# Tony-Tseng/deep-rawburst-sr

Hardware: AMD Instinct MI355X
Metric: bursts/sec 14x48x48 RAW->4x (SyntheticBurstVal shape), DBSR forward (higher is better)
Workload: dtype fp16; 1 GPU; configs[1]: SyntheticBurstVal 14-frame 48x48 -> 384x384 (sr x8 of RAW, x4 of full-res), batch 8 per GPU, full PWC-Net + warp + fusion + decoder; global_batch=8, frames=14, height=48, width=48, out_size=384, parallelism=dp1 (independent bursts per rank), hip_graph=True, fusion_weights_written=True

## Files before the change

### deep-rawburst-sr_amd/csrc/conv2d.hip

```cpp
#include "conv_core.hpp"

#include <algorithm>
#include <type_traits>
#include <cstdlib>
#include <cstring>
#include <vector>

using namespace dbsr;

namespace {

int g_tiled_enabled = 1;

const dbsr_conv_desc* sel_view(const dbsr_conv_desc* d, dbsr_conv_desc& v) {
    if (d->plan_h <= 0 || d->plan_h == d->out_h) return d;
    v = *d;
    v.in_h = d->in_h + (d->plan_h - d->out_h) * d->stride;
    v.out_h = d->plan_h;
    return &v;
}

__host__ __device__ __forceinline__ int pipe_lane_ch(int cb, int h, int g, int cout) {
    const int c = cb + 32 * h + 8 * g;
    return c < cout ? c : cb;
// ... 1513 lines not shown
            asm volatile("ds_read_b128 %0, %1 offset:%2" : "=v"(v) : "v"(a), "i"(16 * (c * S::CH_U4 + 4 * imm)));
            bq[n % AHEAD].v = v;
        };
        auto epilogue = [&](auto y_) {
            constexpr int y = decltype(y_)::value;
            if (has_res) asm volatile("" : "+v"(resv[y]));
            if constexpr (has_gate) asm volatile("" : "+v"(gatev[y]));
            float v[8];
#pragma unroll
            for (int r = 0; r < 4; ++r) {
                v[r] = act1(acc[0][y][r] + bias0[r]);
                v[4 + r] = act1(acc[1][y][r] + bias1[r]);
            }
            if (has_res) {
#pragma unroll
                for (int e = 0; e < 4; ++e) {
                    v[2 * e] = act2(v[2 * e] + H16<T>::lo(resv[y][e]));
                    v[2 * e + 1] = act2(v[2 * e + 1] + H16<T>::hi(resv[y][e]));
                }
            }
            if constexpr (has_gate) {
#pragma unroll
                for (int e = 0; e < 4; ++e) {
                    v[2 * e] = H16<T>::lo(gatev[y][e]) > 0.f ? v[2 * e] : 0.f;
                    v[2 * e + 1] = H16<T>::hi(gatev[y][e]) > 0.f ? v[2 * e + 1] : 0.f;
                }
            }
            u32x4_t o;
#pragma unroll
            for (int e = 0; e < 4; ++e) o[e] = H16<T>::pack(v[2 * e], v[2 * e + 1]);
            __builtin_amdgcn_raw_buffer_store_b128(o, y_rsrc, cout_ok ? ys + y * ys_row : BUF_OOB, 0, 0);
        };

        StaticFor<0, AHEAD>::run([&](auto n_) { rd(n_); });
        StaticFor<0, S::READS>::run([&](auto n_) {
            constexpr int n = decltype(n_)::value, c = S::read_chunk(n);
            constexpr int newer = AHEAD - 1 < S::READS - 1 - n ? AHEAD - 1 : S::READS - 1 - n;
            bf16x8_t v = bq[n % AHEAD].v;
            asm volatile("s_waitcnt lgkmcnt(%1)" : "+v"(v) : "i"(newer));
            Frag<T> bf;
            bf.v = v;
            StaticFor<0, 3>::run([&](auto ky_) {
                constexpr int ky = decltype(ky_)::value;
                if constexpr (S::feeds(n, ky)) {
                    constexpr int y = S::read_row(n) - ky, tap = 3 * ky + S::read_kx(n);
                    const f32x4_t z = {0.f, 0.f, 0.f, 0.f};
                    acc[0][y] = mma(wr[c][tap][0], bf, S::kstep(n, ky) == 0 ? z : acc[0][y]);
                    acc[1][y] = mma(wr[c][tap][1], bf, S::kstep(n, ky) == 0 ? z : acc[1][y]);
                }
            });
            if constexpr (n + AHEAD < S::READS) rd(std::integral_constant<int, n + AHEAD>{});
            StaticFor<0, S::PER>::run([&](auto it_) {
                constexpr int it = decltype(it_)::value;
                if constexpr (n == S::dma_at(it)) {
                    if (more) dma(it, nxt, buf ^ 1);
                }
            });
            StaticFor<0, RPW>::run([&](auto y_) {
                constexpr int y = decltype(y_)::value;
                if constexpr (n == S::res_at(y)) {
                    if (has_res)
                        resv[y] = __builtin_amdgcn_raw_buffer_load_b128(
                            buf_rsrc((const T*)k.r + cur.r_off, rframe_bytes), r_tile + y * r_row, 0, 0);
                    if constexpr (has_gate)
                        gatev[y] = *(const u32x4_t*)((const T*)k.gt + cur.g_off + gl + y * g_row);
                }
                if constexpr (n == S::row_done(y)) epilogue(y_);
            });
        });
        PIPE_STAMP(7 + ti * 5);
        cur = nxt;
#pragma unroll
        for (int rho = 0; rho < 8; ++rho)
            ba[rho] += buf ? (unsigned)(-S::STAGE_U4 * 16) : (unsigned)(S::STAGE_U4 * 16);
    }
    vm_drain();
    PIPE_STAMP(1);
}

template <typename T, int WM, int TW, int TH, int NCH, int EPI>
__global__ __launch_bounds__(512, 1) void conv3x3_ws_kernel(ConvK k, int tiles_x, int tiles_y, int nct, int nsp,
                                                            int px) {
    constexpr bool rows = WM == wsr::WM && !(TH == 16 && NCH == 2 && (EPI == 0 || EPI == 5));
    if constexpr (rows) {
        static_assert(TW == wsr::TW, "the 64-cout tiles are 16 pixels wide");
        ws_rows_body<T, TH, NCH, EPI>(k, tiles_x, tiles_y, nct, nsp, px);
    } else {
        ws_tile_body<T, WM, TW, TH, NCH, EPI>(k, tiles_x, tiles_y, nct, nsp, px);
    }
}

int g_ws_enabled = 1;
inline bool ws_narrow(const dbsr_conv_desc* d) { return d->cout <= 32; }
inline bool ws_short(const dbsr_conv_desc* d) {
    if (d->gate.ptr && d->cout > 32 && d->cin > 32) return true;
    return !ws_narrow(d) && d->cin > 32 && d->out_w % 16 == 0 && d->out_h % 16 == 0 &&
           (long long)d->n_frames * (d->out_w / 16) * (d->out_h / 16) * ((d->cout + 63) / 64) < 128;
}
int pick_ws(const dbsr_conv_desc* d, const dbsr_conv_desc* g) {
    if (!g_ws_enabled || !conv3x3_16(d) || !slices_aligned8(d) || d->cin <= 16 || d->cin > 64 || d->cout % 8 ||
        d->cout > 512)
        return 0;
    const bool narrow = ws_narrow(d);
    const int tw = narrow ? 64 : 16, th = (narrow || ws_short(d)) ? 8 : 16, wm = narrow ? 32 : 64;
    if (narrow && (d->cout < 16 || d->cin > 32)) return 0;
    if (d->out_w % tw || d->out_h % th) return 0;
    if ((long long)d->in_h * d->in_w * d->x.ld * 2 >= (1LL << 31)) return 0;
    if (d->res.ptr && (long long)d->out_h * d->out_w * d->res.ld * 2 >= (1LL << 31)) return 0;
    if (!narrow && 16LL * d->out_w * d->y.ld * 2 >= (1LL << 31)) return 0;
    const int nct = (d->cout + wm - 1) / wm;
    const long long nsp = (long long)d->n_frames * (d->out_w / tw) * (d->out_h / th);
    const int cus = d->max_blocks > 0 ? std::min(d->max_blocks, num_cus()) : num_cus();
    if (cus / 8 / nct < 1 || nsp * nct < 64) return 0;
    if (g->out_h % th) return -1;
    const long long nsp_g = (long long)g->n_frames * (g->out_w / tw) * (g->out_h / th);
    const long long want = (nsp_g + 7) / 8;
    const long long spx = std::max<long long>(1, std::min<long long>(cus / 8 / nct, want));
    return (int)(spx * nct);
}

template <typename T, int WM, int TW, int TH, int NCH>
int launch_ws(const ConvK& k, const dbsr_conv_desc* d, int px, hipStream_t s) {
    const int tiles_x = k.out_w / TW, tiles_y = k.out_h / TH;
    const int nct = (k.cout + WM - 1) / WM;
    const int nsp = d->n_frames * tiles_x * tiles_y;
#define DBSR_WS_LAUNCH(E)                                                                                       \
    hipLaunchKernelGGL((conv3x3_ws_kernel<T, WM, TW, TH, NCH, E>), dim3(8 * px), dim3(512), 0, s, k, tiles_x,    \
                       tiles_y, nct, nsp, px)
    switch (epi_code(k)) {
        case 1: DBSR_WS_LAUNCH(1); break;
        case 2: DBSR_WS_LAUNCH(2); break;
        case 3: DBSR_WS_LAUNCH(3); break;
        case 5: DBSR_WS_LAUNCH(5); break;
        default: DBSR_WS_LAUNCH(0); break;
    }
#undef DBSR_WS_LAUNCH
    DBSR_LAUNCH_CHECK();
    return 0;
}

int g_ks128_enabled = 1;
bool use_ks128(const dbsr_conv_desc* d) {
    if (!g_ks128_enabled || !conv3x3_16(d) || !slices_aligned8(d) || cin_pad(d->cin) != 128 || d->cout != 128)
        return false;
    if (d->out_w % ks128::TW || d->out_h % ks128::TH || (d->plan_h > 0 && d->plan_h != d->out_h)) return false;
    if ((long long)d->in_h * d->in_w * d->x.ld * 2 >= (1LL << 31)) return false;
    return (long long)d->n_frames * (d->out_w / ks128::TW) * (d->out_h / ks128::TH) >= 128;
}
int launch_ks128(const ConvK& k, const dbsr_conv_desc* d, hipStream_t s) {
    return ks128_launch(k, d->n_frames, d->x.dtype == DBSR_F16, epi_code(k), k.max_blocks, num_cus(), s);
}

namespace rbk {
constexpr int TW = 32, TH = 16;
constexpr int MW = TW + 2, MH = TH + 2, MPX = MW * MH;
constexpr int IW = TW + 4, IH = TH + 4, IPX = IW * IH;
constexpr int IN_PIECES = (IPX + 15) / 16;
constexpr int IN_U4 = IN_PIECES * 64;
constexpr int G1 = (MPX + 15) / 16;
constexpr int MID_U4 = G1 * 16 * 4;
constexpr int G2 = TW * TH / 16;
constexpr int NW = 8;
constexpr int PER = (IN_PIECES + NW - 1) / NW;
constexpr int Q1 = (G1 + NW - 1) / NW;
constexpr int Q2 = G2 / NW;
constexpr int NG = 2;
constexpr int LDS_BYTES = (2 * IN_U4 + MID_U4) * 16 + 64 * 4;
static_assert(LDS_BYTES <= 160 * 1024, "resblock LDS");
}

template <typename T, bool HEAD>
__global__ __launch_bounds__(512, 1) void resblock32_kernel(ConvK k1, ConvK k2, int tiles_x, int tiles_y,
                                                            int ntiles) {
    using namespace rbk;
    DBSR_OWN_SIMDS();
    __shared__ __attribute__((aligned(16))) u32x4_t lds[2 * IN_U4 + MID_U4 + 16 + 34];
    u32x4_t* lmid = lds + 2 * IN_U4;
    float* lbias = (float*)(lds + 2 * IN_U4 + MID_U4);
    float* lhead = lbias + 64;
    const int lane = threadIdx.x & 63, wave = __builtin_amdgcn_readfirstlane(threadIdx.x >> 6);
    const int H = k1.in_h, W = k1.in_w;

    Frag<T> w1[9][2], w2[9][2];
#pragma unroll
    for (int tap = 0; tap < 9; ++tap)
#pragma unroll
        for (int h = 0; h < 2; ++h) {
            w1[tap][h].load((const T*)((const char*)k1.w_pipe + (h * 9 + tap) * 1024 + lane * 16));
            w2[tap][h].load((const T*)((const char*)k2.w_pipe + (h * 9 + tap) * 1024 + lane * 16));
        }
    if (threadIdx.x < 64) {
        const ConvK& kb = threadIdx.x < 32 ? k1 : k2;
        lbias[threadIdx.x] = kb.bias ? kb.bias[threadIdx.x & 31] : 0.f;
    }
    if constexpr (HEAD) {
        if (threadIdx.x < 128) lhead[threadIdx.x] = (int)threadIdx.x < k2.head_cout * 32 ? k2.head_w[threadIdx.x] : 0.f;
        if (threadIdx.x < 4)
            lhead[128 + threadIdx.x] = (k2.head_b && (int)threadIdx.x < k2.head_cout) ? k2.head_b[threadIdx.x] : 0.f;
    }

    struct Tile { const T* xf; long long y_off; int y0, x0; };
    auto decode = [&](int i) {
        const int t = rb_tile(i, blockIdx.x, gridDim.x, ntiles);
        Tile tl;
        const int tx = t % tiles_x, r = t / tiles_x, ty = r % tiles_y, f = r / tiles_y;
        tl.y0 = ty * TH; tl.x0 = tx * TW;
        tl.xf = (const T*)k1.x + map_frame(k1.xm, f) * k1.x_is;
        tl.y_off = HEAD ? map_frame(k2.ym, f) * k2.y_is + (long long)tl.y0 * W + tl.x0
                        : map_frame(k2.ym, f) * k2.y_is + k2.y_c0 + ((long long)tl.y0 * W + tl.x0) * k2.y_ld;
        return tl;
    };
    const int my_tiles = ntiles / (int)gridDim.x + ((int)blockIdx.x < ntiles % (int)gridDim.x ? 1 : 0);
    const int pix_b = k1.x_ld * (int)sizeof(T);
    const unsigned frame_bytes = (unsigned)((long long)H * W * pix_b);
    const unsigned lds0 = (unsigned)(unsigned long long)(__attribute__((address_space(3))) u32x4_t*)lds;
    auto dma = [&](const Tile& tl, int buf) {
        int ln = lane;
        asm volatile("" : "+v"(ln));
#pragma unroll
        for (int it = 0; it < PER; ++it) {
            const int piece = min(wave + NW * it, IN_PIECES - 1);
            const int p = piece * 16 + (ln >> 2), ph = ln & 3;
            const int gg = 2 * ((ph & 1) ^ ((p >> 2) & 1)) + (ph >> 1);
            const int r = p / IW, c = p - r * IW;
            const int hy = tl.y0 - 2 + r, hx = tl.x0 - 2 + c;
            const bool ok = p < IPX && (unsigned)hy < (unsigned)H && (unsigned)hx < (unsigned)W;
            lds_dma16(tl.xf, frame_bytes, ok ? (hy * W + hx) * pix_b + gg * 16 : BUF_OOB, 0,
                      lds0 + (buf * IN_U4 + piece * 64) * 16);
        }
    };

    auto taps = [&](const u32x4_t* img, int iw, int g, const auto& P0, const Frag<T> (&w)[9][2], auto& acc) {
        constexpr int NB = std::extent<std::remove_reference_t<decltype(P0)>>::value;
        int bs[NB][8];
#pragma unroll
        for (int j = 0; j < NB; ++j)
#pragma unroll
            for (int rho = 0; rho < 8; ++rho) bs[j][rho] = 4 * P0[j] + halo_phys(P0[j] + rho, g);
        Frag<T> bq[NB][3];
        auto rd = [&](int j, int tap) {
            const int imm = (tap / 3) * iw + tap % 3;
            Frag<T> b;
            b.v = __builtin_bit_cast(bf16x8_t, img[bs[j][imm & 7] + 4 * imm]);
            return b;
        };
#pragma unroll
        for (int j = 0; j < NB; ++j) {
            bq[j][0] = rd(j, 0);
            bq[j][1] = rd(j, 1);
        }
        StaticFor<0, 9>::run([&](auto t_) {
            constexpr int tap = decltype(t_)::value;
            const f32x4_t z = {0.f, 0.f, 0.f, 0.f};
#pragma unroll
            for (int j = 0; j < NB; ++j) {
                acc[j][0] = mma(w[tap][0], bq[j][tap % 3], tap == 0 ? z : acc[j][0]);
                acc[j][1] = mma(w[tap][1], bq[j][tap % 3], tap == 0 ? z : acc[j][1]);
                if constexpr (tap + 2 < 9) bq[j][(tap + 2) % 3] = rd(j, tap + 2);
            }
        });
        __builtin_amdgcn_iglp_opt(0);
    };

    auto store_out = [&](const Tile& tl, int i, int g, int col, const u32x4_t& o) {
        const int q = wave + NW * i;
        const long long px = (long long)(q >> 1) * W + 16 * (q & 1) + col;
        if constexpr (HEAD) {
            if (g < k2.head_cout) ((float*)k2.y)[tl.y_off + px + (long long)g * H * W] = __uint_as_float(o[0]);
        } else {
            *(u32x4_t*)((T*)k2.y + tl.y_off + px * k2.y_ld + 8 * g) = o;
        }
    };
    Tile cur = decode(0), prev = cur;
    if (my_tiles > 0) dma(cur, 0);
    u32x4_t outv[Q2];
    for (int ti = 0; ti < my_tiles; ++ti) {
        dma_barrier();
        int ln = lane;
        asm volatile("" : "+v"(ln));
        const int g = ln >> 4, col = ln & 15;
        if (ti > 0) {
#pragma unroll
            for (int i = 0; i < Q2; ++i) store_out(prev, i, g, col, outv[i]);
        }
        const u32x4_t* lin = lds + (ti & 1) * IN_U4;
        const bool more = ti + 1 < my_tiles;
        const Tile nxt = more ? decode(ti + 1) : cur;
        if (more) dma(nxt, (ti + 1) & 1);
        {
            const float4 b0 = *(const float4*)(lbias + 8 * g), b1 = *(const float4*)(lbias + 8 * g + 4);
            const float bv[8] = {b0.x, b0.y, b0.z, b0.w, b1.x, b1.y, b1.z, b1.w};
            auto conv1 = [&](auto nb_, auto q0_) {
                constexpr int NB = decltype(nb_)::value, Q0 = decltype(q0_)::value;
                int pa[NB], P0[NB];
#pragma unroll
                for (int j = 0; j < NB; ++j) {
                    pa[j] = min(16 * (wave + NW * (Q0 + j)) + col, MPX - 1);
                    const int r = pa[j] / MW, c = pa[j] - r * MW;
                    P0[j] = r * IW + c;
                }
                f32x4_t acc[NB][2];
                taps(lin, IW, g, P0, w1, acc);
#pragma unroll
                for (int j = 0; j < NB; ++j) {
                    const int p = 16 * (wave + NW * (Q0 + j)) + col;
                    const int r = pa[j] / MW, c = pa[j] - r * MW;
                    const int fy = cur.y0 - 1 + r, fx = cur.x0 - 1 + c;
                    const bool inside = (unsigned)fy < (unsigned)H && (unsigned)fx < (unsigned)W;
                    u32x4_t o;
#pragma unroll
                    for (int e = 0; e < 2; ++e) {
                        o[e] = relu16x2(H16<T>::pack(acc[j][0][2 * e] + bv[2 * e], acc[j][0][2 * e + 1] + bv[2 * e + 1]));
                        o[2 + e] = relu16x2(H16<T>::pack(acc[j][1][2 * e] + bv[4 + 2 * e],
                                                         acc[j][1][2 * e + 1] + bv[4 + 2 * e + 1]));
                    }
                    if (!inside) o = u32x4_t{0u, 0u, 0u, 0u};
                    if (p < MPX) lmid[4 * p + halo_phys(p, g)] = o;
                }
            };
            StaticFor<0, Q1 / NG>::run([&](auto bt_) {
                conv1(std::integral_constant<int, NG>{}, std::integral_constant<int, NG * decltype(bt_)::value>{});
            });
            if constexpr (Q1 % NG != 0) {
                if (wave + NW * (Q1 - Q1 % NG) < G1)
                    conv1(std::integral_constant<int, Q1 % NG>{}, std::integral_constant<int, Q1 - Q1 % NG>{});
            }
        }
        dma_barrier();
        {
            const float4 b0 = *(const float4*)(lbias + 32 + 8 * g), b1 = *(const float4*)(lbias + 32 + 8 * g + 4);
            const float bv[8] = {b0.x, b0.y, b0.z, b0.w, b1.x, b1.y, b1.z, b1.w};
            StaticFor<0, Q2 / NG>::run([&](auto bt_) {
                constexpr int bt = decltype(bt_)::value;
                int row[NG], cc[NG], P0[NG];
#pragma unroll
                for (int j = 0; j < NG; ++j) {
                    const int q = wave + NW * (NG * bt + j);
                    row[j] = q >> 1;
                    cc[j] = 16 * (q & 1) + col;
                    P0[j] = row[j] * MW + cc[j];
                }
                f32x4_t acc[NG][2];
                taps(lmid, MW, g, P0, w2, acc);
#pragma unroll
                for (int j = 0; j < NG; ++j) {
                    const int PR = (row[j] + 2) * IW + cc[j] + 2;
                    const u32x4_t rq = lin[4 * PR + halo_phys(PR, g)];
                    float v[8];
#pragma unroll
                    for (int r = 0; r < 4; ++r) {
                        v[r] = acc[j][0][r] + bv[r];
                        v[4 + r] = acc[j][1][r] + bv[4 + r];
                    }
                    u32x4_t o;
                    if constexpr (HEAD) {
#pragma unroll
                        for (int e = 0; e < 4; ++e) {
                            v[2 * e] = fmaxf(v[2 * e] + H16<T>::lo(rq[e]), 0.f);
                            v[2 * e + 1] = fmaxf(v[2 * e + 1] + H16<T>::hi(rq[e]), 0.f);
                        }
                        float hs[4];
#pragma unroll
                        for (int c = 0; c < 4; ++c) {
                            const float4 w0 = *(const float4*)(lhead + c * 32 + 8 * g);
                            const float4 w1 = *(const float4*)(lhead + c * 32 + 8 * g + 4);
                            float a = v[0] * w0.x;
                            a = fmaf(v[1], w0.y, a); a = fmaf(v[2], w0.z, a); a = fmaf(v[3], w0.w, a);
                            a = fmaf(v[4], w1.x, a); a = fmaf(v[5], w1.y, a); a = fmaf(v[6], w1.z, a);
                            a = fmaf(v[7], w1.w, a);
                            a += __shfl_xor(a, 16, 64);
                            a += __shfl_xor(a, 32, 64);
                            hs[c] = a;
                        }
                        const float hv = g == 0 ? hs[0] : g == 1 ? hs[1] : g == 2 ? hs[2] : hs[3];
                        o = u32x4_t{__float_as_uint(fmaxf(hv + lhead[128 + g], 0.f)), 0u, 0u, 0u};
                    } else {
#pragma unroll
                        for (int e = 0; e < 4; ++e)
                            o[e] = relu16x2(H16<T>::pack(v[2 * e] + H16<T>::lo(rq[e]), v[2 * e + 1] + H16<T>::hi(rq[e])));
                    }
                    outv[NG * bt + j] = o;
                }
            });
        }
        prev = cur;
        cur = nxt;
    }
    if (my_tiles > 0) {
#pragma unroll
        for (int i = 0; i < Q2; ++i) store_out(prev, i, lane >> 4, lane & 15, outv[i]);
    }
    vm_drain();
}

void tensor_span(const dbsr_tensor& t, int n, long long per_img, int es, unsigned long long& lo,
                 unsigned long long& hi) {
    long long mn = 0, mx = 0;
    for (int f = 0; f < n; ++f) {
        const long long img = (long long)(f / t.map.fpg) * t.map.group_stride + t.map.group_offset +
                              (long long)(f % t.map.fpg) * t.map.inner_stride;
        if (f == 0 || img < mn) mn = img;
        if (f == 0 || img > mx) mx = img;
    }
    const unsigned long long base = (unsigned long long)(uintptr_t)t.ptr;
    lo = base + (unsigned long long)((mn * t.img_stride + t.c0) * es);
    hi = base + (unsigned long long)((mx * t.img_stride + per_img) * es);
}
bool resblock_out_disjoint(const dbsr_conv_desc* c1, const dbsr_conv_desc* c2, const dbsr_tensor* head_out,
                           int head_cout) {
    const long long hw = (long long)c1->in_h * c1->in_w;
    const int C = c1->cin;
    unsigned long long xl, xh, yl, yh;
    tensor_span(c1->x, c1->n_frames, (hw - 1) * c1->x.ld + c1->x.c0 + C, 2, xl, xh);
    if (head_out) tensor_span(*head_out, c1->n_frames, (long long)head_cout * hw, 4, yl, yh);
    else tensor_span(c2->y, c1->n_frames, (hw - 1) * c2->y.ld + c2->y.c0 + C, 2, yl, yh);
    return yh <= xl || xh <= yl;
}

int resblock_channels(const dbsr_conv_desc* c1, const dbsr_conv_desc* c2) {
    if (!c1 || !c2) return 0;
    const int C = c1->cin;
    if (C != 32 && C != 64) return 0;
    auto conv_ok = [C](const dbsr_conv_desc* d) {
        return is16(d->x.dtype) && d->y.dtype == d->x.dtype && !d->precise && d->kh == 3 && d->kw == 3 &&
               d->stride == 1 && d->pad == 1 && d->dil == 1 && d->cin == C && d->cout == C &&
               d->out_mode == DBSR_OUT_NHWC && !d->gate.ptr && d->in_h == d->out_h && d->in_w == d->out_w;
    };
    if (!conv_ok(c1) || !conv_ok(c2)) return 0;
    if (c1->act != DBSR_ACT_RELU || c1->res.ptr || c2->act != DBSR_ACT_NONE || c2->post_act != DBSR_ACT_RELU)
        return 0;
    if (c2->res.ptr != c1->x.ptr || c2->res.c0 != c1->x.c0 || c2->res.ld != c1->x.ld ||
        c2->res.img_stride != c1->x.img_stride || c2->res.dtype != c1->x.dtype ||
        std::memcmp(&c2->res.map, &c1->x.map, sizeof(dbsr_frame_map)) != 0)
        return 0;
    if (c1->n_frames != c2->n_frames || c1->in_h != c2->in_h || c1->in_w != c2->in_w || c1->x.dtype != c2->y.dtype)
        return 0;
    if (C == 32 ? (c1->in_w % rbk::TW || c1->in_h % rbk::TH) : (c1->in_w % rb64::TW || c1->in_h % rb64::TH)) return 0;
    if (C == 64) {
        const long long tiles = (long long)c1->n_frames * (c1->in_w / rb64::TW) * (c1->in_h / rb64::TH);
        const int cus = c1->max_blocks > 0 ? std::min(c1->max_blocks, num_cus()) : num_cus();
        if (tiles > 2LL * cus) return 0;
    }
    if (c1->x.ld % 8 || c1->x.c0 % 8 || c1->x.c0 + C > c1->x.ld) return 0;
    if (c2->y.ld % 8 || c2->y.c0 % 8 || c2->y.c0 + C > c2->y.ld) return 0;
    return (long long)c1->in_h * c1->in_w * c1->x.ld * 2 < (1LL << 31) ? C : 0;
}

template <typename T, int MT, int NT, typename XT = T>
int launch_conv(const ConvK& k0, hipStream_t s) {
    ConvK k = k0;
    k.stage_epi = MT * NT >= 2 && sizeof(T) == 2 && sizeof(XT) == 2 && k.ksplit == 1 &&
                  k.out_mode == DBSR_OUT_NHWC && !k.y_f32 && !k.r && !k.gt && k.cout % 8 == 0 && k.y_ld % 8 == 0 &&
                  k.y_c0 % 8 == 0 && k.head_cout == 0;
    dim3 grid((k.npix + 4 * NT * 16 - 1) / (4 * NT * 16), (k.cout + MT * 16 - 1) / (MT * 16), k.ksplit);
    hipLaunchKernelGGL((conv2d_kernel<T, MT, NT, XT>), grid, dim3(256), 0, s, k);
    DBSR_LAUNCH_CHECK();
    if (k.ksplit > 1) {
        const long long n = (long long)k.npix * (k.cw / 4);
        hipLaunchKernelGGL((conv_splitk_finalize<T>), dim3((unsigned)((n + 255) / 256)), dim3(256), 0, s, k);
        DBSR_LAUNCH_CHECK();
    }
    return 0;
}

int choose_ksplit(const ConvK& k, int mt, int nt) {
    const long long blocks = (long long)((k.npix + 64 * nt - 1) / (64 * nt)) * ((k.cout + 16 * mt - 1) / (16 * mt));
    const int nks = k.KGp >> 2;
    const long long target = nks >= 64 ? 1024 : 512;
    if (blocks >= target / 2 || nks < 16) return 1;
    int sp = (int)((target + blocks - 1) / blocks);
    sp = std::min(sp, nks / 8);
    sp = std::min(sp, 32);
    return std::max(sp, 1);
}
size_t splitk_bytes(const dbsr_conv_desc* d, int sp) {
    const int npix = (int)((long long)d->n_frames * d->out_h * d->out_w);
    return sp > 1 ? (size_t)sp * npix * round_up(d->cout, 4) * sizeof(float) : 0;
}
void pick_generic_tile(const ConvK& k, int& best_m, int& best_n) {
    const int mts[3] = {4, 2, 1}, nts[3] = {4, 2, 1};
    const long long minb = 512;
    best_m = 1;
    best_n = 1;
    for (int a = 0; a < 3; ++a) {
        if (mts[a] > 1 && k.cout <= (mts[a] / 2) * 16) continue;
        for (int b = 0; b < 3; ++b) {
            const long long blocks = (long long)((k.npix + 64 * nts[b] - 1) / (64 * nts[b])) *
                                     ((k.cout + 16 * mts[a] - 1) / (16 * mts[a]));
            if (blocks >= minb) {
                best_m = mts[a];
                best_n = nts[b];
                return;
            }
        }
    }
}

template <typename T>
__global__ __launch_bounds__(256) void conv3x3_small_kernel(ConvK k, int groups_x, long long ngroups) {
    const int lane = threadIdx.x & 63, g = lane >> 4, col = lane & 15;
    const int nco = k.cout / 16;
    Frag<T> a[4][3];
    f32x4_t bias[4];
#pragma unroll
    for (int b = 0; b < 4; ++b) {
        bias[b] = load_bias4(k, min(b, nco - 1) * 16 + g * 4);
#pragma unroll
        for (int st = 0; st < 3; ++st)
            a[b][st].load((const T*)k.w + (long long)(min(b, nco - 1) * 16 + col) * k.Kp + 32 * st + 8 * g);
    }
    const long long wave0 = ((long long)blockIdx.x * blockDim.x + threadIdx.x) >> 6;
    const long long nwaves = ((long long)gridDim.x * blockDim.x) >> 6;
    for (long long gi = wave0; gi < ngroups; gi += nwaves) {
        const int gx = (int)(gi % groups_x);
        const long long r = gi / groups_x;
        const int y = (int)(r % k.out_h), f = (int)(r / k.out_h);
        const int x = gx * 16 + col;
        const T* xf = (const T*)k.x + map_frame(k.xm, f) * k.x_is;
        Frag<T> bq[3];
#pragma unroll
        for (int st = 0; st < 3; ++st) {
            const int tap = 4 * st + g, ky = tap / 3, kx = tap - 3 * (tap / 3);
            const int iy = y + ky - 1, ix = x + kx - 1;
            if (tap < 9 && (unsigned)iy < (unsigned)k.in_h && (unsigned)ix < (unsigned)k.in_w)
                bq[st].load(xf + ((long long)iy * k.in_w + ix) * k.x_ld);
            else
                bq[st].zero();
        }
        f32x4_t acc[4];
#pragma unroll
        for (int b = 0; b < 4; ++b) {
            acc[b] = f32x4_t{0.f, 0.f, 0.f, 0.f};
#pragma unroll
            for (int st = 0; st < 3; ++st) acc[b] = mma(a[b][st], bq[st], acc[b]);
        }
        if (x < k.out_w) {
            T* yp = (T*)k.y + map_frame(k.ym, f) * k.y_is + k.y_c0 + ((long long)y * k.out_w + x) * k.y_ld + 4 * g;
#pragma unroll
            for (int b = 0; b < 4; ++b) {
                if (b >= nco) break;
                uint2 o;
                o.x = H16<T>::pack(apply_act(acc[b][0] + bias[b][0], k.act), apply_act(acc[b][1] + bias[b][1], k.act));
                o.y = H16<T>::pack(apply_act(acc[b][2] + bias[b][2], k.act), apply_act(acc[b][3] + bias[b][3], k.act));
                *(uint2*)(yp + 16 * b) = o;
            }
// ... 1008 lines not shown
```

### deep-rawburst-sr_amd/csrc/conv_core.hpp

```cpp
#pragma once
#include "common.hpp"
#include "ks128_sched.hpp"
#include "ws_sched.hpp"

#include <vector>

namespace dbsr {

inline int round_up(int a, int b) { return (a + b - 1) / b * b; }
inline int cin_pad(int cin) { return cin <= 16 ? round_up(cin, 8) : round_up(cin, 32); }


inline bool is16(int dtype) { return dtype == DBSR_BF16 || dtype == DBSR_F16; }
inline int esize(int dtype) { return is16(dtype) ? 2 : 4; }


struct ConvK {
    const void* x; long long x_is; int x_ld; dbsr_frame_map xm; int in_h, in_w;
    const void* w; const float* bias; int Kp, KG, KGp, CG, kw, stride, pad, dil, cout;
    void* y; int y_f32; long long y_is; int y_ld, y_c0; dbsr_frame_map ym; int out_h, out_w;
    int act;
    const void* r; long long r_is; int r_ld, r_c0; dbsr_frame_map rm; int post_act;
    const void* gt; long long g_is; int g_ld, g_c0; dbsr_frame_map gm;
    int out_mode, shuffle, cps;
    int npix;
    int vec_store;
    int ksplit;
    float* ws;
    int cw;
    const void* w_pipe;
    int max_blocks;
    const float* head_w;
    const float* head_b;
    int head_cout;
    int stage_epi;
};

template <typename T> struct Frag;
template <> struct Frag<bf16_t> {
    bf16x8_t v;
    __device__ __forceinline__ void load(const bf16_t* p) { v = *(const bf16x8_t*)p; }
    __device__ __forceinline__ void zero() { v = bf16x8_t{0, 0, 0, 0, 0, 0, 0, 0}; }
};
template <> struct Frag<f16_t> {
    bf16x8_t v;
    __device__ __forceinline__ void load(const f16_t* p) { v = *(const bf16x8_t*)p; }
    __device__ __forceinline__ void zero() { v = bf16x8_t{0, 0, 0, 0, 0, 0, 0, 0}; }
};
template <> struct Frag<float> {
    float4 a, b;
    __device__ __forceinline__ void load(const float* p) { a = *(const float4*)p; b = *(const float4*)(p + 4); }
    __device__ __forceinline__ void load(const bf16_t* p) {
        const u32x4_t q = *(const u32x4_t*)p;
        a = make_float4(__uint_as_float(q[0] << 16), __uint_as_float(q[0] & 0xffff0000u),
                        __uint_as_float(q[1] << 16), __uint_as_float(q[1] & 0xffff0000u));
        b = make_float4(__uint_as_float(q[2] << 16), __uint_as_float(q[2] & 0xffff0000u),
                        __uint_as_float(q[3] << 16), __uint_as_float(q[3] & 0xffff0000u));
    }
    __device__ __forceinline__ void load(const f16_t* p) {
        const u32x4_t q = *(const u32x4_t*)p;
        a = make_float4(H16<f16_t>::lo(q[0]), H16<f16_t>::hi(q[0]), H16<f16_t>::lo(q[1]), H16<f16_t>::hi(q[1]));
        b = make_float4(H16<f16_t>::lo(q[2]), H16<f16_t>::hi(q[2]), H16<f16_t>::lo(q[3]), H16<f16_t>::hi(q[3]));
    }
    __device__ __forceinline__ void zero() { a = make_float4(0, 0, 0, 0); b = a; }
};

__device__ __forceinline__ f32x4_t mma(const Frag<bf16_t>& A, const Frag<bf16_t>& B, f32x4_t c) {
    typedef __attribute__((ext_vector_type(8))) __bf16 bfv;
    return __builtin_amdgcn_mfma_f32_16x16x32_bf16(__builtin_bit_cast(bfv, A.v), __builtin_bit_cast(bfv, B.v), c,
                                                   0, 0, 0);
}
__device__ __forceinline__ f32x4_t mma(const Frag<f16_t>& A, const Frag<f16_t>& B, f32x4_t c) {
    typedef __attribute__((ext_vector_type(8))) _Float16 hv;
    return __builtin_amdgcn_mfma_f32_16x16x32_f16(__builtin_bit_cast(hv, A.v), __builtin_bit_cast(hv, B.v), c, 0, 0, 0);
}
__device__ __forceinline__ f32x4_t mma(const Frag<float>& A, const Frag<float>& B, f32x4_t c) {
    c = __builtin_amdgcn_mfma_f32_16x16x4f32(A.a.x, B.a.x, c, 0, 0, 0);
    c = __builtin_amdgcn_mfma_f32_16x16x4f32(A.a.y, B.a.y, c, 0, 0, 0);
    c = __builtin_amdgcn_mfma_f32_16x16x4f32(A.a.z, B.a.z, c, 0, 0, 0);
    c = __builtin_amdgcn_mfma_f32_16x16x4f32(A.a.w, B.a.w, c, 0, 0, 0);
    c = __builtin_amdgcn_mfma_f32_16x16x4f32(A.b.x, B.b.x, c, 0, 0, 0);
    c = __builtin_amdgcn_mfma_f32_16x16x4f32(A.b.y, B.b.y, c, 0, 0, 0);
    c = __builtin_amdgcn_mfma_f32_16x16x4f32(A.b.z, B.b.z, c, 0, 0, 0);
    c = __builtin_amdgcn_mfma_f32_16x16x4f32(A.b.w, B.b.w, c, 0, 0, 0);
    return c;
}


__device__ __forceinline__ unsigned relu16x2(unsigned v) {
    typedef short s16x2 __attribute__((ext_vector_type(2)));
    return __builtin_bit_cast(unsigned, __builtin_elementwise_max(__builtin_bit_cast(s16x2, v), s16x2{0, 0}));
}
__device__ __forceinline__ int halo_phys(int p, int g) { return 2 * (g & 1) + ((g >> 1) ^ ((p >> 2) & 1)); }


__host__ __device__ __forceinline__ int rb_tile(int i, int b, int nb, int ntiles) {
    if (nb == 256 && (i + 1) * 256 <= ntiles) return i * 256 + (b & 7) * 32 + (b >> 3);
    return i * nb + b;
}


inline bool rb_mapping_ok(int nb, int ntiles) {
    std::vector<unsigned char> seen(ntiles, 0);
    for (int b = 0; b < nb; ++b) {
        const int my = ntiles / nb + (b < ntiles % nb ? 1 : 0);
        for (int i = 0; i < my; ++i) {
            const int t = rb_tile(i, b, nb, ntiles);
            if (t < 0 || t >= ntiles || seen[t]) return false;
            seen[t] = 1;
        }
    }
    return true;
}

int resblock64_launch(const ConvK& k1, const ConvK& k2, int n_frames, bool f16, int max_blocks, int cus,
                      hipStream_t s);
namespace rb64 {
constexpr int TW = 16, TH = 8;
}

int ks128_launch(const ConvK& k, int n_frames, bool f16, int epi, int max_blocks, int cus, hipStream_t s);

}
```

Measured before the change: 3474 bursts/s.

## Restructure resblock32 kernel into per-wave row-rolling bands with fused stores

Reworks the fused two-conv residual block kernel so each wave owns a column strip and a band of rows. Input fragments are read once and fed to the MFMAs of up to three output rows via a row-rolling schedule, instead of re-reading all nine taps per pixel group. A small edge pass covers the leftover halo columns, LDS reads use explicit ds_read_b128 with a fixed lookahead and waitcnt, and outputs are written straight from the conv2 epilogue rather than buffered to the next iteration. This aims to cut LDS read traffic and register pressure, at the cost of a more complex hand-built schedule and uneven per-wave work.

```diff
diff --git a/deep-rawburst-sr_amd/csrc/conv2d.hip b/deep-rawburst-sr_amd/csrc/conv2d.hip
--- a/deep-rawburst-sr_amd/csrc/conv2d.hip
+++ b/deep-rawburst-sr_amd/csrc/conv2d.hip
@@ -1689,21 +1689,7 @@
 }
 
 namespace rbk {
-constexpr int TW = 32, TH = 16;
-constexpr int MW = TW + 2, MH = TH + 2, MPX = MW * MH;
-constexpr int IW = TW + 4, IH = TH + 4, IPX = IW * IH;
-constexpr int IN_PIECES = (IPX + 15) / 16;
-constexpr int IN_U4 = IN_PIECES * 64;
-constexpr int G1 = (MPX + 15) / 16;
-constexpr int MID_U4 = G1 * 16 * 4;
-constexpr int G2 = TW * TH / 16;
-constexpr int NW = 8;
-constexpr int PER = (IN_PIECES + NW - 1) / NW;
-constexpr int Q1 = (G1 + NW - 1) / NW;
-constexpr int Q2 = G2 / NW;
-constexpr int NG = 2;
-constexpr int LDS_BYTES = (2 * IN_U4 + MID_U4) * 16 + 64 * 4;
-static_assert(LDS_BYTES <= 160 * 1024, "resblock LDS");
+using namespace rb32;
 }
 
 template <typename T, bool HEAD>
@@ -1716,6 +1702,7 @@
     float* lbias = (float*)(lds + 2 * IN_U4 + MID_U4);
     float* lhead = lbias + 64;
     const int lane = threadIdx.x & 63, wave = __builtin_amdgcn_readfirstlane(threadIdx.x >> 6);
+    const int strip = wave_strip(wave), band = wave_band(wave);
     const int H = k1.in_h, W = k1.in_w;
 
     Frag<T> w1[9][2], w2[9][2];
@@ -1751,6 +1738,7 @@
     const int pix_b = k1.x_ld * (int)sizeof(T);
     const unsigned frame_bytes = (unsigned)((long long)H * W * pix_b);
     const unsigned lds0 = (unsigned)(unsigned long long)(__attribute__((address_space(3))) u32x4_t*)lds;
+    const unsigned lmid_b = lds0 + 2 * IN_U4 * 16;
     auto dma = [&](const Tile& tl, int buf) {
         int ln = lane;
         asm volatile("" : "+v"(ln));
@@ -1767,167 +1755,229 @@
         }
     };
 
-    auto taps = [&](const u32x4_t* img, int iw, int g, const auto& P0, const Frag<T> (&w)[9][2], auto& acc) {
-        constexpr int NB = std::extent<std::remove_reference_t<decltype(P0)>>::value;
-        int bs[NB][8];
-#pragma unroll
-        for (int j = 0; j < NB; ++j)
-#pragma unroll
-            for (int rho = 0; rho < 8; ++rho) bs[j][rho] = 4 * P0[j] + halo_phys(P0[j] + rho, g);
-        Frag<T> bq[NB][3];
-        auto rd = [&](int j, int tap) {
-            const int imm = (tap / 3) * iw + tap % 3;
-            Frag<T> b;
-            b.v = __builtin_bit_cast(bf16x8_t, img[bs[j][imm & 7] + 4 * imm]);
-            return b;
+    auto bases = [&](unsigned img, int P0, int g, unsigned (&ba)[8]) {
+#pragma unroll
+        for (int rho = 0; rho < 8; ++rho) ba[rho] = img + 16u * (4 * P0 + halo_phys(P0 + rho, g));
+    };
+    auto mid_pack = [&](const f32x4_t& a0, const f32x4_t& a1, const float (&bv)[8]) {
+        u32x4_t o;
+#pragma unroll
+        for (int e = 0; e < 2; ++e) {
+            o[e] = relu16x2(H16<T>::pack(a0[2 * e] + bv[2 * e], a0[2 * e + 1] + bv[2 * e + 1]));
+            o[2 + e] = relu16x2(H16<T>::pack(a1[2 * e] + bv[4 + 2 * e], a1[2 * e + 1] + bv[4 + 2 * e + 1]));
+        }
+        return o;
+    };
+
+    auto conv1_band = [&](auto nr_, int R0, unsigned lin_b, const Tile& tl, int g, int col, const float (&bv)[8]) {
+        constexpr int NR = decltype(nr_)::value;
+        using S = Rows<NR>;
+        const int c0 = 16 * strip + col;
+        unsigned ba[8];
+        bases(lin_b, R0 * IW + c0, g, ba);
+        const bool col_in = (unsigned)(tl.x0 - 1 + c0) < (unsigned)W;
+        f32x4_t acc[2][NR];
+        Frag<T> bq[AHEAD];
+        auto rd = [&](auto n_) {
+            constexpr int n = decltype(n_)::value, imm = rows_pix<NR>(n, IW);
+            const unsigned a = ba[imm & 7];
+            bf16x8_t v;
+            asm volatile("ds_read_b128 %0, %1 offset:%2" : "=v"(v) : "v"(a), "i"(64 * imm));
+            bq[n % AHEAD].v = v;
         };
-#pragma unroll
-        for (int j = 0; j < NB; ++j) {
-            bq[j][0] = rd(j, 0);
-            bq[j][1] = rd(j, 1);
-        }
-        StaticFor<0, 9>::run([&](auto t_) {
-            constexpr int tap = decltype(t_)::value;
+        StaticFor<0, AHEAD>::run([&](auto n_) { rd(n_); });
+        StaticFor<0, S::READS>::run([&](auto n_) {
+            constexpr int n = decltype(n_)::value;
+            constexpr int newer = AHEAD - 1 < S::READS - 1 - n ? AHEAD - 1 : S::READS - 1 - n;
+            bf16x8_t v = bq[n % AHEAD].v;
+            asm volatile("s_waitcnt lgkmcnt(%1)" : "+v"(v) : "i"(newer));
+            Frag<T> bf;
+            bf.v = v;
+            StaticFor<0, 3>::run([&](auto ky_) {
+                constexpr int ky = decltype(ky_)::value;
+                if constexpr (S::feeds(n, ky)) {
+                    constexpr int r = S::read_row(n) - ky, tap = S::tap(n, ky);
+                    const f32x4_t z = {0.f, 0.f, 0.f, 0.f};
+                    acc[0][r] = mma(w1[tap][0], bf, tap == 0 ? z : acc[0][r]);
+                    acc[1][r] = mma(w1[tap][1], bf, tap == 0 ? z : acc[1][r]);
+                }
+            });
+            if constexpr (n + AHEAD < S::READS) rd(std::integral_constant<int, n + AHEAD>{});
+            StaticFor<0, NR>::run([&](auto r_) {
+                constexpr int r = decltype(r_)::value;
+                if constexpr (n == S::row_done(r)) {
+                    const int p = (R0 + r) * MW + c0;
+                    const bool inside = col_in && (unsigned)(tl.y0 - 1 + R0 + r) < (unsigned)H;
+                    u32x4_t o = mid_pack(acc[0][r], acc[1][r], bv);
+                    if (!inside) o = u32x4_t{0u, 0u, 0u, 0u};
+                    lmid[4 * p + halo_phys(p, g)] = o;
+                }
+            });
+        });
+    };
+    auto conv1_edge = [&](int eg, unsigned lin_b, const Tile& tl, int g, int col, const float (&bv)[8]) {
+        const int e = min(16 * eg + col, EDGE_PX - 1);
+        const int r = edge_row(e), c = edge_col(e);
+        unsigned ba[8];
+        bases(lin_b, r * IW + c, g, ba);
+        f32x4_t acc[2];
+        Frag<T> bq[AHEAD];
+        auto rd = [&](auto n_) {
+            constexpr int n = decltype(n_)::value, imm = edge_pix(n);
+            const unsigned a = ba[imm & 7];
+            bf16x8_t v;
+            asm volatile("ds_read_b128 %0, %1 offset:%2" : "=v"(v) : "v"(a), "i"(64 * imm));
+            bq[n % AHEAD].v = v;
+        };
+        StaticFor<0, AHEAD>::run([&](auto n_) { rd(n_); });
+        StaticFor<0, EDGE_READS>::run([&](auto n_) {
+            constexpr int n = decltype(n_)::value;
+            constexpr int newer = AHEAD - 1 < EDGE_READS - 1 - n ? AHEAD - 1 : EDGE_READS - 1 - n;
+            bf16x8_t v = bq[n % AHEAD].v;
+            asm volatile("s_waitcnt lgkmcnt(%1)" : "+v"(v) : "i"(newer));
+            Frag<T> bf;
+            bf.v = v;
             const f32x4_t z = {0.f, 0.f, 0.f, 0.f};
-#pragma unroll
-            for (int j = 0; j < NB; ++j) {
-                acc[j][0] = mma(w[tap][0], bq[j][tap % 3], tap == 0 ? z : acc[j][0]);
-                acc[j][1] = mma(w[tap][1], bq[j][tap % 3], tap == 0 ? z : acc[j][1]);
-                if constexpr (tap + 2 < 9) bq[j][(tap + 2) % 3] = rd(j, tap + 2);
-            }
+            acc[0] = mma(w1[n][0], bf, n == 0 ? z : acc[0]);
+            acc[1] = mma(w1[n][1], bf, n == 0 ? z : acc[1]);
+            if constexpr (n + AHEAD < EDGE_READS) rd(std::integral_constant<int, n + AHEAD>{});
         });
-        __builtin_amdgcn_iglp_opt(0);
-    };
-
-    auto store_out = [&](const Tile& tl, int i, int g, int col, const u32x4_t& o) {
-        const int q = wave + NW * i;
-        const long long px = (long long)(q >> 1) * W + 16 * (q & 1) + col;
-        if constexpr (HEAD) {
-            if (g < k2.head_cout) ((float*)k2.y)[tl.y_off + px + (long long)g * H * W] = __uint_as_float(o[0]);
-        } else {
-            *(u32x4_t*)((T*)k2.y + tl.y_off + px * k2.y_ld + 8 * g) = o;
-        }
-    };
-    Tile cur = decode(0), prev = cur;
+        const int p = r * MW + c;
+        const bool inside = (unsigned)(tl.y0 - 1 + r) < (unsigned)H && (unsigned)(tl.x0 - 1 + c) < (unsigned)W;
+        u32x4_t o = mid_pack(acc[0], acc[1], bv);
+        if (!inside) o = u32x4_t{0u, 0u, 0u, 0u};
+        if (16 * eg + col < EDGE_PX) lmid[4 * p + halo_phys(p, g)] = o;
+    };
+    auto conv2_band = [&](unsigned lin_b, const Tile& tl, int g, int col, const float (&bv)[8]) {
+        using S = Conv2;
+        constexpr int NR = S::NR;
+        const int c0 = 16 * strip + col, R0 = NR * band;
+        unsigned ba[8], br[8];
+        bases(lmid_b, R0 * MW + c0, g, ba);
+        bases(lin_b, (R0 + 2) * IW + c0 + 2, g, br);
+        const long long px0 = (long long)R0 * W + c0;
+        f32x4_t acc[2][NR];
+        Frag<T> bq[AHEAD];
+        auto rd = [&](auto n_) {
+            constexpr int n = decltype(n_)::value;
+            constexpr int imm = S::is_res(n) ? S::res_row(n) * IW : rows_pix<NR>(S::frag(n), MW);
+            const unsigned a = S::is_res(n) ? br[imm & 7] : ba[imm & 7];
+            bf16x8_t v;
+            asm volatile("ds_read_b128 %0, %1 offset:%2" : "=v"(v) : "v"(a), "i"(64 * imm));
+            bq[n % AHEAD].v = v;
+        };
+        auto epilogue = [&](auto y_, const u32x4_t& rq) {
+            constexpr int y = decltype(y_)::value;
+            float v[8];
+#pragma unroll
+            for (int r = 0; r < 4; ++r) {
+                v[r] = acc[0][y][r] + bv[r];
+                v[4 + r] = acc[1][y][r] + bv[4 + r];
+            }
+            const long long px = px0 + (long long)y * W;
+            if constexpr (HEAD) {
+#pragma unroll
+                for (int e = 0; e < 4; ++e) {
+                    v[2 * e] = fmaxf(v[2 * e] + H16<T>::lo(rq[e]), 0.f);
+                    v[2 * e + 1] = fmaxf(v[2 * e + 1] + H16<T>::hi(rq[e]), 0.f);
+                }
+                float hs[4];
+#pragma unroll
+                for (int c = 0; c < 4; ++c) {
+                    const float4 w0 = *(const float4*)(lhead + c * 32 + 8 * g);
+                    const float4 w4 = *(const float4*)(lhead + c * 32 + 8 * g + 4);
+                    float a = v[0] * w0.x;
+                    a = fmaf(v[1], w0.y, a); a = fmaf(v[2], w0.z, a); a = fmaf(v[3], w0.w, a);
+                    a = fmaf(v[4], w4.x, a); a = fmaf(v[5], w4.y, a); a = fmaf(v[6], w4.z, a);
+                    a = fmaf(v[7], w4.w, a);
+                    a += __shfl_xor(a, 16, 64);
+                    a += __shfl_xor(a, 32, 64);
+                    hs[c] = a;
+                }
+                const float hv = g == 0 ? hs[0] : g == 1 ? hs[1] : g == 2 ? hs[2] : hs[3];
+                if (g < k2.head_cout)
+                    ((float*)k2.y)[tl.y_off + px + (long long)g * H * W] = fmaxf(hv + lhead[128 + g], 0.f);
+            } else {
+                u32x4_t o;
+#pragma unroll
+                for (int e = 0; e < 4; ++e)
+                    o[e] = relu16x2(H16<T>::pack(v[2 * e] + H16<T>::lo(rq[e]), v[2 * e + 1] + H16<T>::hi(rq[e])));
+                *(u32x4_t*)((T*)k2.y + tl.y_off + px * k2.y_ld + 8 * g) = o;
+            }
+        };
+        StaticFor<0, AHEAD>::run([&](auto n_) { rd(n_); });
+        StaticFor<0, S::ITEMS>::run([&](auto n_) {
+            constexpr int n = decltype(n_)::value;
+            constexpr int newer = AHEAD - 1 < S::ITEMS - 1 - n ? AHEAD - 1 : S::ITEMS - 1 - n;
+            bf16x8_t v = bq[n % AHEAD].v;
+            asm volatile("s_waitcnt lgkmcnt(%1)" : "+v"(v) : "i"(newer));
+            if constexpr (S::is_res(n)) {
+                epilogue(std::integral_constant<int, S::res_row(n)>{}, __builtin_bit_cast(u32x4_t, v));
+            } else {
+                constexpr int f = S::frag(n);
+                Frag<T> bf;
+                bf.v = v;
+                StaticFor<0, 3>::run([&](auto ky_) {
+                    constexpr int ky = decltype(ky_)::value;
+                    if constexpr (Rows<NR>::feeds(f, ky)) {
+                        constexpr int r = Rows<NR>::read_row(f) - ky, tap = Rows<NR>::tap(f, ky);
+                        const f32x4_t z = {0.f, 0.f, 0.f, 0.f};
+                        acc[0][r] = mma(w2[tap][0], bf, tap == 0 ? z : acc[0][r]);
+                        acc[1][r] = mma(w2[tap][1], bf, tap == 0 ? z : acc[1][r]);
+                    }
+                });
+            }
+            if constexpr (n + AHEAD < S::ITEMS) rd(std::integral_constant<int, n + AHEAD>{});
+        });
+    };
+    auto bias8 = [&](const float* b, int g, float (&bv)[8]) {
+        const float4 b0 = *(const float4*)(b + 8 * g), b1 = *(const float4*)(b + 8 * g + 4);
+        bv[0] = b0.x; bv[1] = b0.y; bv[2] = b0.z; bv[3] = b0.w;
+        bv[4] = b1.x; bv[5] = b1.y; bv[6] = b1.z; bv[7] = b1.w;
+#pragma unroll
+        for (int i = 0; i < 8; ++i) asm volatile("" : "+v"(bv[i]));
+    };
+
+    PIPE_STAMP(0);
+    Tile cur = decode(0);
     if (my_tiles > 0) dma(cur, 0);
-    u32x4_t outv[Q2];
+    vm_drain();
+    PIPE_STAMP(2);
     for (int ti = 0; ti < my_tiles; ++ti) {
-        dma_barrier();
+        PIPE_STAMP(3 + ti * 5);
+        DBSR_VM_WAIT(STORES);
+        __syncthreads();
+        PIPE_STAMP(4 + ti * 5);
         int ln = lane;
         asm volatile("" : "+v"(ln));
         const int g = ln >> 4, col = ln & 15;
-        if (ti > 0) {
-#pragma unroll
-            for (int i = 0; i < Q2; ++i) store_out(prev, i, g, col, outv[i]);
-        }
-        const u32x4_t* lin = lds + (ti & 1) * IN_U4;
+        const unsigned lin_b = lds0 + (ti & 1) * IN_U4 * 16;
         const bool more = ti + 1 < my_tiles;
         const Tile nxt = more ? decode(ti + 1) : cur;
         if (more) dma(nxt, (ti + 1) & 1);
         {
-            const float4 b0 = *(const float4*)(lbias + 8 * g), b1 = *(const float4*)(lbias + 8 * g + 4);
-            const float bv[8] = {b0.x, b0.y, b0.z, b0.w, b1.x, b1.y, b1.z, b1.w};
-            auto conv1 = [&](auto nb_, auto q0_) {
-                constexpr int NB = decltype(nb_)::value, Q0 = decltype(q0_)::value;
-                int pa[NB], P0[NB];
-#pragma unroll
-                for (int j = 0; j < NB; ++j) {
-                    pa[j] = min(16 * (wave + NW * (Q0 + j)) + col, MPX - 1);
-                    const int r = pa[j] / MW, c = pa[j] - r * MW;
-                    P0[j] = r * IW + c;
-                }
-                f32x4_t acc[NB][2];
-                taps(lin, IW, g, P0, w1, acc);
-#pragma unroll
-                for (int j = 0; j < NB; ++j) {
-                    const int p = 16 * (wave + NW * (Q0 + j)) + col;
-                    const int r = pa[j] / MW, c = pa[j] - r * MW;
-                    const int fy = cur.y0 - 1 + r, fx = cur.x0 - 1 + c;
-                    const bool inside = (unsigned)fy < (unsigned)H && (unsigned)fx < (unsigned)W;
-                    u32x4_t o;
-#pragma unroll
-                    for (int e = 0; e < 2; ++e) {
-                        o[e] = relu16x2(H16<T>::pack(acc[j][0][2 * e] + bv[2 * e], acc[j][0][2 * e + 1] + bv[2 * e + 1]));
-                        o[2 + e] = relu16x2(H16<T>::pack(acc[j][1][2 * e] + bv[4 + 2 * e],
-                                                         acc[j][1][2 * e + 1] + bv[4 + 2 * e + 1]));
-                    }
-                    if (!inside) o = u32x4_t{0u, 0u, 0u, 0u};
-                    if (p < MPX) lmid[4 * p + halo_phys(p, g)] = o;
-                }
-            };
-            StaticFor<0, Q1 / NG>::run([&](auto bt_) {
-                conv1(std::integral_constant<int, NG>{}, std::integral_constant<int, NG * decltype(bt_)::value>{});
-            });
-            if constexpr (Q1 % NG != 0) {
-                if (wave + NW * (Q1 - Q1 % NG) < G1)
-                    conv1(std::integral_constant<int, Q1 % NG>{}, std::integral_constant<int, Q1 - Q1 % NG>{});
-            }
-        }
+            float bv[8];
+            bias8(lbias, g, bv);
+            if (c1_rows(band) == 5) {
+                conv1_band(std::integral_constant<int, 5>{}, c1_row0(band), lin_b, cur, g, col, bv);
+            } else {
+                conv1_band(std::integral_constant<int, 4>{}, c1_row0(band), lin_b, cur, g, col, bv);
+                if (edge_group(wave) >= 0) conv1_edge(edge_group(wave), lin_b, cur, g, col, bv);
+            }
+        }
+        PIPE_STAMP(5 + ti * 5);
         dma_barrier();
+        PIPE_STAMP(6 + ti * 5);
         {
-            const float4 b0 = *(const float4*)(lbias + 32 + 8 * g), b1 = *(const float4*)(lbias + 32 + 8 * g + 4);
-            const float bv[8] = {b0.x, b0.y, b0.z, b0.w, b1.x, b1.y, b1.z, b1.w};
-            StaticFor<0, Q2 / NG>::run([&](auto bt_) {
-                constexpr int bt = decltype(bt_)::value;
-                int row[NG], cc[NG], P0[NG];
-#pragma unroll
-                for (int j = 0; j < NG; ++j) {
-                    const int q = wave + NW * (NG * bt + j);
-                    row[j] = q >> 1;
-                    cc[j] = 16 * (q & 1) + col;
-                    P0[j] = row[j] * MW + cc[j];
-                }
-                f32x4_t acc[NG][2];
-                taps(lmid, MW, g, P0, w2, acc);
-#pragma unroll
-                for (int j = 0; j < NG; ++j) {
-                    const int PR = (row[j] + 2) * IW + cc[j] + 2;
-                    const u32x4_t rq = lin[4 * PR + halo_phys(PR, g)];
-                    float v[8];
-#pragma unroll
-                    for (int r = 0; r < 4; ++r) {
-                        v[r] = acc[j][0][r] + bv[r];
-                        v[4 + r] = acc[j][1][r] + bv[4 + r];
-                    }
-                    u32x4_t o;
-                    if constexpr (HEAD) {
-#pragma unroll
-                        for (int e = 0; e < 4; ++e) {
-                            v[2 * e] = fmaxf(v[2 * e] + H16<T>::lo(rq[e]), 0.f);
-                            v[2 * e + 1] = fmaxf(v[2 * e + 1] + H16<T>::hi(rq[e]), 0.f);
-                        }
-                        float hs[4];
-#pragma unroll
-                        for (int c = 0; c < 4; ++c) {
-                            const float4 w0 = *(const float4*)(lhead + c * 32 + 8 * g);
-                            const float4 w1 = *(const float4*)(lhead + c * 32 + 8 * g + 4);
-                            float a = v[0] * w0.x;
-                            a = fmaf(v[1], w0.y, a); a = fmaf(v[2], w0.z, a); a = fmaf(v[3], w0.w, a);
-                            a = fmaf(v[4], w1.x, a); a = fmaf(v[5], w1.y, a); a = fmaf(v[6], w1.z, a);
-                            a = fmaf(v[7], w1.w, a);
-                            a += __shfl_xor(a, 16, 64);
-                            a += __shfl_xor(a, 32, 64);
-                            hs[c] = a;
-                        }
-                        const float hv = g == 0 ? hs[0] : g == 1 ? hs[1] : g == 2 ? hs[2] : hs[3];
-                        o = u32x4_t{__float_as_uint(fmaxf(hv + lhead[128 + g], 0.f)), 0u, 0u, 0u};
-                    } else {
-#pragma unroll
-                        for (int e = 0; e < 4; ++e)
-                            o[e] = relu16x2(H16<T>::pack(v[2 * e] + H16<T>::lo(rq[e]), v[2 * e + 1] + H16<T>::hi(rq[e])));
-                    }
-                    outv[NG * bt + j] = o;
-                }
-            });
-        }
-        prev = cur;
+            float bv[8];
+            bias8(lbias + 32, g, bv);
+            conv2_band(lin_b, cur, g, col, bv);
+        }
+        PIPE_STAMP(7 + ti * 5);
         cur = nxt;
     }
-    if (my_tiles > 0) {
-#pragma unroll
-        for (int i = 0; i < Q2; ++i) store_out(prev, i, lane >> 4, lane & 15, outv[i]);
-    }
     vm_drain();
+    PIPE_STAMP(1);
 }
 
 void tensor_span(const dbsr_tensor& t, int n, long long per_img, int es, unsigned long long& lo,
diff --git a/deep-rawburst-sr_amd/csrc/conv_core.hpp b/deep-rawburst-sr_amd/csrc/conv_core.hpp
--- a/deep-rawburst-sr_amd/csrc/conv_core.hpp
+++ b/deep-rawburst-sr_amd/csrc/conv_core.hpp
@@ -2,6 +2,7 @@
 #include "common.hpp"
 #include "ks128_sched.hpp"
 #include "ws_sched.hpp"
+#include "rb32_sched.hpp"
 
 #include <vector>
 
diff --git a/deep-rawburst-sr_amd/csrc/rb32_sched.hpp b/deep-rawburst-sr_amd/csrc/rb32_sched.hpp
--- /dev/null
+++ b/deep-rawburst-sr_amd/csrc/rb32_sched.hpp
@@ -0,0 +1,104 @@
+#pragma once
+#include "ks128_sched.hpp"
+
+namespace dbsr {
+namespace rb32 {
+
+constexpr int TW = 32, TH = 16;
+constexpr int MW = TW + 2, MH = TH + 2, MPX = MW * MH;
+constexpr int IW = TW + 4, IH = TH + 4, IPX = IW * IH;
+constexpr int IN_PIECES = (IPX + 15) / 16;
+constexpr int IN_U4 = IN_PIECES * 64;
+constexpr int MID_U4 = (MPX + 15) / 16 * 16 * 4;
+constexpr int NW = 8, NS = 2, NB = 4;
+constexpr int PER = (IN_PIECES + NW - 1) / NW;
+constexpr int AHEAD = 4;
+constexpr int LDS_BYTES = (2 * IN_U4 + MID_U4) * 16 + 64 * 4;
+static_assert(LDS_BYTES <= 160 * 1024, "resblock LDS");
+
+using ks128::frag_slot;
+using ks128::piece_kgroup;
+
+constexpr int wave_strip(int w) { return w & 1; }
+constexpr int wave_band(int w) { return w >> 1; }
+
+constexpr int c1_rows(int b) { return b < 2 ? 5 : 4; }
+constexpr int c1_row0(int b) { return b < 2 ? 5 * b : 10 + 4 * (b - 2); }
+static_assert(c1_row0(NB - 1) + c1_rows(NB - 1) == MH, "conv1 bands cover the intermediate's rows");
+
+template <int NR_>
+struct Rows {
+    static constexpr int NR = NR_;
+    static constexpr int READS = (NR + 2) * 3;
+    static constexpr int MFMAS = NR * 9 * 2;
+    static constexpr int read_row(int n) { return n / 3; }
+    static constexpr int read_kx(int n) { return n % 3; }
+    static constexpr bool feeds(int n, int ky) { return read_row(n) - ky >= 0 && read_row(n) - ky < NR; }
+    static constexpr int tap(int n, int ky) { return 3 * ky + read_kx(n); }
+    static constexpr int row_done(int r) { return (r + 2) * 3 + 2; }
+    static constexpr bool schedule_ok() {
+        int next[NR] = {}, total = 0;
+        for (int n = 0; n < READS; ++n)
+            for (int ky = 0; ky < 3; ++ky)
+                if (feeds(n, ky)) {
+                    const int r = read_row(n) - ky;
+                    if (tap(n, ky) != next[r] || n > row_done(r)) return false;
+                    ++next[r];
+                    total += 2;
+                }
+        for (int r = 0; r < NR; ++r)
+            if (next[r] != 9 || row_done(r) >= READS) return false;
+        return total == MFMAS && row_done(NR - 1) == READS - 1 && AHEAD >= 1 && AHEAD < READS;
+    }
+};
+static_assert(Rows<5>::schedule_ok() && Rows<4>::schedule_ok(), "conv1 row-rolling schedule");
+template <int NR> constexpr int rows_pix(int n, int iw) { return Rows<NR>::read_row(n) * iw + Rows<NR>::read_kx(n); }
+
+constexpr int EDGE_PX = 2 * MH, EDGE_GROUPS = (EDGE_PX + 15) / 16;
+constexpr int edge_group(int w) { return c1_rows(wave_band(w)) == 4 && w - 2 * NS < EDGE_GROUPS ? w - 2 * NS : -1; }
+constexpr int edge_row(int e) { return e % MH; }
+constexpr int edge_col(int e) { return TW + e / MH; }
+constexpr int EDGE_READS = 9, EDGE_MFMAS = 18;
+constexpr int edge_pix(int tap) { return (tap / 3) * IW + tap % 3; }
+
+constexpr int c1_reads(int w) { return (c1_rows(wave_band(w)) + 2) * 3 + (edge_group(w) >= 0 ? EDGE_READS : 0); }
+constexpr int c1_mfmas(int w) { return c1_rows(wave_band(w)) * 18 + (edge_group(w) >= 0 ? EDGE_MFMAS : 0); }
+constexpr bool conv1_ok() {
+    int total = 0, groups = 0;
+    for (int w = 0; w < NW; ++w) {
+        if (c1_mfmas(w) > 90) return false;
+        total += c1_mfmas(w);
+        groups += edge_group(w) >= 0;
+    }
+    return total == (MPX + 15) / 16 * 18 && groups == EDGE_GROUPS;
+}
+static_assert(conv1_ok(), "conv1 work split");
+
+struct Conv2 {
+    static constexpr int NR = TH / NB;
+    static constexpr int FRAGS = (NR + 2) * 3, ITEMS = FRAGS + NR, MFMAS = NR * 18;
+    static constexpr bool is_res(int n) { return n >= 9 && (n - 9) % 4 == 0; }
+    static constexpr int res_row(int n) { return (n - 9) / 4; }
+    static constexpr int frag(int n) { return n < 9 ? n : 9 + 3 * ((n - 9) / 4) + (n - 9) % 4 - 1; }
+    static constexpr int epilogue_at(int y) { return 9 + 4 * y; }
+    static constexpr bool schedule_ok() {
+        int nf = 0, nr = 0;
+        for (int n = 0; n < ITEMS; ++n) {
+            if (is_res(n)) {
+                if (res_row(n) != nr || n != epilogue_at(nr) || n == 0 || is_res(n - 1) ||
+                    frag(n - 1) != Rows<NR>::row_done(nr))
+                    return false;
+                ++nr;
+            } else {
+                if (frag(n) != nf) return false;
+                ++nf;
+            }
+        }
+        return nf == FRAGS && nr == NR && is_res(ITEMS - 1) && AHEAD < ITEMS;
+    }
+};
+static_assert(Conv2::schedule_ok(), "conv2 row-rolling schedule");
+constexpr int STORES = Conv2::NR;
+
+}
+}
```

Result: faster. 3523 bursts/s, median of 6 (+1.4%).
